# valida-xyz/valida

Measured on NVIDIA H100. Metric: trace rows/sec proven (Fibonacci), higher is better.
Workload: dtype u32 (BabyBear, 31-bit modular) + ext5

## Files before the change

### valida_b200/csrc/bb.cuh

```cuda
#pragma once
#include <cstdint>
#include <cuda_runtime.h>

namespace bb {

constexpr uint32_t P = 0x78000001u;
constexpr uint32_t PINV = 0x88000001u;
constexpr uint32_t R1 = 0x0ffffffeu;
constexpr uint32_t R2 = 1172168163u;
constexpr uint32_t GEN_CANON = 31;

#ifdef __CUDACC__
#define BB_HD __host__ __device__ __forceinline__
#else
#define BB_HD inline
#endif

BB_HD uint32_t umin32(uint32_t a, uint32_t b) { return a < b ? a : b; }
BB_HD uint32_t add(uint32_t a, uint32_t b) { uint32_t s = a + b; return umin32(s, s - P); }
BB_HD uint32_t sub(uint32_t a, uint32_t b) { uint32_t d = a - b; return umin32(d, d + P); }
BB_HD uint32_t neg(uint32_t a) { return a ? P - a : 0; }
BB_HD uint32_t dbl(uint32_t a) { return add(a, a); }
BB_HD uint32_t mul(uint32_t a, uint32_t b) {
    uint64_t t = (uint64_t)a * b;
    uint32_t m = (uint32_t)t * PINV;
#ifdef __CUDA_ARCH__
    uint32_t u = (uint32_t)(t >> 32) - __umulhi(m, P);
#else
    uint32_t u = (uint32_t)(t >> 32) - (uint32_t)(((uint64_t)m * P) >> 32);
#endif
    return umin32(u, u + P);
}
BB_HD uint32_t sqr(uint32_t a) { return mul(a, a); }
BB_HD uint32_t to_monty(uint32_t canonical) { return mul(canonical, R2); }
BB_HD uint32_t from_monty(uint32_t m) { return mul(m, 1u); }
BB_HD uint32_t pow(uint32_t a_monty, uint64_t e) {
    uint32_t r = R1;
    while (e) { if (e & 1) r = mul(r, a_monty); a_monty = mul(a_monty, a_monty); e >>= 1; }
    return r;
}
BB_HD uint32_t inv(uint32_t a_monty) { return pow(a_monty, P - 2); }

struct E5 { uint32_t c[5]; };
BB_HD E5 e5_zero() { E5 r; for (int i = 0; i < 5; i++) r.c[i] = 0; return r; }
BB_HD E5 e5_one() { E5 r = e5_zero(); r.c[0] = R1; return r; }
BB_HD E5 e5_from_base(uint32_t b) { E5 r = e5_zero(); r.c[0] = b; return r; }
BB_HD bool e5_is_zero(const E5& a) { return (a.c[0] | a.c[1] | a.c[2] | a.c[3] | a.c[4]) == 0; }
BB_HD E5 e5_add(const E5& a, const E5& b) { E5 r; for (int i = 0; i < 5; i++) r.c[i] = add(a.c[i], b.c[i]); return r; }
BB_HD E5 e5_sub(const E5& a, const E5& b) { E5 r; for (int i = 0; i < 5; i++) r.c[i] = sub(a.c[i], b.c[i]); return r; }
BB_HD E5 e5_neg(const E5& a) { E5 r; for (int i = 0; i < 5; i++) r.c[i] = neg(a.c[i]); return r; }
BB_HD E5 e5_add_base(const E5& a, uint32_t b) { E5 r = a; r.c[0] = add(r.c[0], b); return r; }
BB_HD E5 e5_sub_base(const E5& a, uint32_t b) { E5 r = a; r.c[0] = sub(r.c[0], b); return r; }
BB_HD E5 e5_mul_base(const E5& a, uint32_t b) { E5 r; for (int i = 0; i < 5; i++) r.c[i] = mul(a.c[i], b); return r; }

BB_HD uint32_t monty_reduce64(uint64_t t) {
    uint32_t hi = (uint32_t)(t >> 32), lo = (uint32_t)t;
    hi = umin32(hi, hi - P); hi = umin32(hi, hi - P);
    uint32_t m = lo * PINV;
#ifdef __CUDA_ARCH__
    uint32_t u = hi - __umulhi(m, P);
#else
    uint32_t u = hi - (uint32_t)(((uint64_t)m * P) >> 32);
#endif
    return umin32(u, u + P);
}

#ifdef __CUDACC__
__device__ __forceinline__ uint64_t madw(uint32_t a, uint32_t b, uint64_t c) {
    uint64_t r;
    asm("mad.wide.u32 %0, %1, %2, %3;" : "=l"(r) : "r"(a), "r"(b), "l"(c));
    return r;
}
__device__ __forceinline__ uint64_t lazy_fold(uint64_t a) { return madw((uint32_t)(a >> 32), R1, (uint64_t)(uint32_t)a); }

struct Lazy5 {
    uint64_t a[5]; int np;
    __device__ __forceinline__ void init() { for (int l = 0; l < 5; l++) a[l] = 0; np = 0; }
    __device__ __forceinline__ void fold() { for (int l = 0; l < 5; l++) a[l] = lazy_fold(a[l]); np = 0; }
    __device__ __forceinline__ void step() { if (np == 4) fold(); np++; }
    __device__ __forceinline__ void fma_base(const E5& x, uint32_t y) {
        step();
#pragma unroll
        for (int l = 0; l < 5; l++) a[l] = madw(x.c[l], y, a[l]);
    }
    __device__ __forceinline__ void fma_ext(const E5& x, const E5& y, const E5& y2) {
#pragma unroll
        for (int r = 0; r < 5; r++) {
            step();
#pragma unroll
            for (int k = 0; k < 5; k++) a[k] = madw(x.c[r], k >= r ? y.c[k - r] : y2.c[k - r + 5], a[k]);
        }
    }
    __device__ __forceinline__ E5 value() const { E5 r; for (int l = 0; l < 5; l++) r.c[l] = monty_reduce64(a[l]); return r; }
};
__device__ __forceinline__ E5 e5_dbl(const E5& a) { E5 r; for (int i = 0; i < 5; i++) r.c[i] = dbl(a.c[i]); return r; }
#endif

BB_HD E5 e5_mul(const E5& a, const E5& b) {
#ifdef __CUDA_ARCH__
    Lazy5 t; t.init(); t.fma_ext(a, b, e5_dbl(b));
    return t.value();
#else
    E5 r;
#define PR(i, j) ((uint64_t)a.c[i] * b.c[j])
    uint32_t l0 = monty_reduce64(PR(0, 0));
    uint32_t l1 = monty_reduce64(PR(0, 1) + PR(1, 0));
    uint32_t l2 = monty_reduce64(PR(0, 2) + PR(1, 1) + PR(2, 0));
    uint32_t l3 = monty_reduce64(PR(0, 3) + PR(1, 2) + PR(2, 1) + PR(3, 0));
    uint32_t l4 = add(monty_reduce64(PR(0, 4) + PR(1, 3) + PR(2, 2) + PR(3, 1)), monty_reduce64(PR(4, 0)));
    uint32_t h0 = monty_reduce64(PR(1, 4) + PR(2, 3) + PR(3, 2) + PR(4, 1));
    uint32_t h1 = monty_reduce64(PR(2, 4) + PR(3, 3) + PR(4, 2));
    uint32_t h2 = monty_reduce64(PR(3, 4) + PR(4, 3));
    uint32_t h3 = monty_reduce64(PR(4, 4));
#undef PR
    r.c[0] = add(l0, dbl(h0));
    r.c[1] = add(l1, dbl(h1));
    r.c[2] = add(l2, dbl(h2));
    r.c[3] = add(l3, dbl(h3));
    r.c[4] = l4;
    return r;
#endif
}
BB_HD E5 e5_sqr(const E5& a) { return e5_mul(a, a); }
BB_HD E5 e5_pow(E5 a, uint64_t e) {
    E5 r = e5_one();
    while (e) { if (e & 1) r = e5_mul(r, a); a = e5_sqr(a); e >>= 1; }
    return r;
}
BB_HD E5 e5_exp_pow2(E5 a, int k) { while (k-- > 0) a = e5_sqr(a); return a; }
BB_HD E5 e5_frobenius(const E5& a, const uint32_t zpow[5]) {
    E5 r; r.c[0] = a.c[0];
    for (int i = 1; i < 5; i++) r.c[i] = mul(a.c[i], zpow[i]);
    return r;
}
BB_HD void e5_frob_consts(uint32_t zpow[5]) {
    uint32_t z = pow(to_monty(2), (P - 1) / 5);
    zpow[0] = R1;
    for (int i = 1; i < 5; i++) zpow[i] = mul(zpow[i - 1], z);
}
BB_HD E5 e5_inv(const E5& a) {
    uint32_t zp[5];
    e5_frob_consts(zp);
    E5 f1 = e5_frobenius(a, zp), f2 = e5_frobenius(f1, zp), f3 = e5_frobenius(f2, zp), f4 = e5_frobenius(f3, zp);
    E5 prod = e5_mul(e5_mul(f1, f2), e5_mul(f3, f4));
    E5 n = e5_mul(a, prod);
    return e5_mul_base(prod, inv(n.c[0]));
}

BB_HD uint32_t reverse_bits(uint32_t x, int bits) {
#ifdef __CUDA_ARCH__
    return bits ? (__brev(x) >> (32 - bits)) : 0;
#else
    uint32_t r = 0;
    for (int i = 0; i < bits; i++) r = (r << 1) | ((x >> i) & 1);
    return r;
#endif
}

BB_HD uint32_t two_adic_generator_monty(int bits) {
    uint32_t g = to_monty(0x1a427a41u);
    for (int i = 0; i < 27 - bits; i++) g = sqr(g);
    return g;
}

}
```

### valida_b200/csrc/ntt.cu

```cuda
#include "ctx.h"
#include <cstdlib>

namespace {

using bb::mul; using bb::add; using bb::sub;

struct PassParams {
    const uint32_t* src; uint32_t* dst;
    uint64_t src_cs, dst_cs;
    uint64_t src_rs, src_gs;
    uint64_t dst_rs, dst_gs;
    uint32_t log_len;
    uint32_t tile;
    uint64_t groups;
    uint32_t inverse;
    uint32_t src_bitrev;
    uint32_t dst_natural;
    uint32_t g_bits;
    uint32_t pre_mode; uint32_t pre_r, pre_g, pre_shift;
    uint32_t post_mode; uint32_t post_shift, post_g, post_k; uint32_t post_scale;
    const uint32_t* root_lo; const uint32_t* root_hi;
    const uint32_t* root3;
    const uint32_t* tab_lo; const uint32_t* tab_hi;
    uint32_t tab_base;
    uint32_t tab_step;
};

__device__ __forceinline__ uint32_t root_pow(const PassParams& p, uint32_t e) {
    const uint32_t a = __ldg(p.root3 + (e & 511)), b = __ldg(p.root3 + 512 + ((e >> 9) & 511)), c = __ldg(p.root3 + 1024 + ((e >> 18) & 511));
    return mul(mul(a, b), c);
}

__device__ __forceinline__ uint32_t pad(uint32_t i) { return i + (i >> 4) + (i >> 9); }

template <int LQ, int RHO>
__device__ __forceinline__ constexpr uint32_t unit_off(uint32_t m) {
    uint32_t o = m << LQ;
    o += (LQ >= 4) ? (m << (LQ >= 4 ? LQ - 4 : 0)) : (m >> (LQ < 4 ? 4 - LQ : 0));
    if (LQ >= 9) o += m << (LQ >= 9 ? LQ - 9 : 0);
    else if (LQ + RHO >= 9) o += m >> (LQ < 9 ? 9 - LQ : 0);
    return o;
}

template <int RHO, int LOG_LEN, int S>
__device__ __forceinline__ void radix_unit(uint32_t* __restrict__ grp, const uint32_t* __restrict__ tw, uint32_t u) {
    constexpr int R = 1 << RHO;
    constexpr int LQ = LOG_LEN - S - RHO;
    constexpr bool IMM = (LQ + RHO >= 4);
    const uint32_t j = u & ((1u << LQ) - 1), blk = u >> LQ;
    const uint32_t base = (blk << (LQ + RHO)) + j;
    uint32_t* const g0 = grp + pad(base);
    uint32_t x[R];
#pragma unroll
    for (int m = 0; m < R; m++) x[m] = IMM ? g0[unit_off<LQ, RHO>(m)] : grp[pad(base + ((uint32_t)m << LQ))];
#pragma unroll
    for (int a = 0; a < RHO; a++) {
        const int half = R >> (a + 1);
        constexpr int E0 = LQ + S;
        const uint32_t tj = j << (S + a);
        const uint32_t* const tw0 = tw + tj + (tj >> 5);
#pragma unroll
        for (int m0 = 0; m0 < R; m0++) {
            if ((m0 & half) == 0) {
                const int m1 = m0 + half, mm = m0 & (half - 1);
                const uint32_t A = x[m0], B = x[m1];
                x[m0] = add(A, B);
                if (a == RHO - 1 && LQ == 0) x[m1] = sub(A, B);
                else {
                    const uint32_t d = A - B + bb::P;
                    uint32_t wv;
                    if (E0 + a >= 5) wv = tw0[((uint32_t)mm << (E0 + a)) + ((uint32_t)mm << (E0 + a >= 5 ? E0 + a - 5 : 0))];
                    else { const uint32_t ti = tj + ((uint32_t)mm << (E0 + a)); wv = tw[ti + (ti >> 5)]; }
                    x[m1] = mul(d, wv);
                }
            }
        }
    }
#pragma unroll
    for (int m = 0; m < R; m++) { if (IMM) g0[unit_off<LQ, RHO>(m)] = x[m]; else grp[pad(base + ((uint32_t)m << LQ))] = x[m]; }
}

template <int RHO, int LOG_LEN, int S>
__device__ __forceinline__ void radix_step(uint32_t* data, const uint32_t* tw, uint32_t T, uint32_t LS, uint32_t tid, uint32_t nt) {
    constexpr int LU = LOG_LEN - RHO;
    const uint32_t total_units = T << LU;
    for (uint32_t w = tid; w < total_units; w += nt) {
        const uint32_t t = w >> LU, u = w & ((1u << LU) - 1);
        radix_unit<RHO, LOG_LEN, S>(data + t * LS, tw, u);
    }
    __syncthreads();
}

template <int LOG_LEN, int S>
__device__ __forceinline__ void all_stages(uint32_t* data, const uint32_t* tw, uint32_t T, uint32_t LS, uint32_t tid, uint32_t nt) {
    if constexpr (LOG_LEN - S >= 4) {
        radix_step<4, LOG_LEN, S>(data, tw, T, LS, tid, nt);
        all_stages<LOG_LEN, S + 4>(data, tw, T, LS, tid, nt);
    } else if constexpr (LOG_LEN - S == 3) {
        radix_step<3, LOG_LEN, S>(data, tw, T, LS, tid, nt);
    } else if constexpr (LOG_LEN - S == 2) {
        radix_step<2, LOG_LEN, S>(data, tw, T, LS, tid, nt);
    } else if constexpr (LOG_LEN - S == 1) {
        radix_step<1, LOG_LEN, S>(data, tw, T, LS, tid, nt);
    }
}

__host__ __device__ constexpr uint32_t cbrev(uint32_t x, int bits) {
    uint32_t r = 0;
    for (int i = 0; i < bits; i++) r |= ((x >> i) & 1u) << (bits - 1 - i);
    return r;
}
template <int LOG_LEN> struct Std {
    static constexpr int LOG_T = 14 - LOG_LEN;
    static constexpr uint32_t T = 1u << (LOG_T > 0 ? LOG_T : 0), L = 1u << LOG_LEN;
    static constexpr uint32_t LS = (L + (L >> 4) + (L >> 9)) | 1;
    static constexpr int LR0 = LOG_LEN - 5;
    static constexpr int LB = LOG_LEN - 9;
};
__device__ __forceinline__ constexpr uint32_t off_b5(uint32_t c) { return c + (c >> 4); }
template <int LR0> __device__ __forceinline__ constexpr uint32_t off_strided(uint32_t k) {
    return (k << LR0) + (LR0 >= 4 ? (k << (LR0 >= 4 ? LR0 - 4 : 0)) : (k >> (LR0 < 4 ? 4 - LR0 : 0))) + (k >> (9 - LR0));
}
template <int LR0> __device__ __forceinline__ uint32_t base_strided(uint32_t r0) { return r0 + (LR0 >= 4 ? (r0 >> 4) : 0u); }
template <int LB> __device__ __forceinline__ uint32_t base_rowrev(uint32_t B) { return (B << LB) + ((B << LB) >> 4) + (B >> (9 - LB)); }
template <int LB> __device__ __forceinline__ constexpr uint32_t off_rowrev(uint32_t c) { return c + (LB >= 4 ? (c >> 4) : 0u); }

template <int LOG_LEN, bool BITREV>
__device__ __forceinline__ void load_strided_std(const PassParams& p, const uint32_t* __restrict__ src, uint32_t* __restrict__ data, uint64_t g0, uint32_t tid) {
    using S = Std<LOG_LEN>;
    const uint32_t tt = tid & (S::T - 1), r0 = tid >> S::LOG_T;
    const uint32_t* g = src + g0 + tt + (uint64_t)r0 * p.src_rs;
    const uint64_t ks = p.src_rs << S::LR0;
    uint32_t* sl;
    if (BITREV) { const uint32_t B = bb::reverse_bits(r0, S::LR0); sl = data + tt * S::LS + (B << 5) + (B << 1) + (B >> 4); }
    else sl = data + tt * S::LS + base_strided<S::LR0>(r0);
#pragma unroll
    for (int kb = 0; kb < 32; kb += 8) {
        uint32_t v[8];
#pragma unroll
        for (int u = 0; u < 8; u++) v[u] = __ldg(g + (uint64_t)(kb + u) * ks);
#pragma unroll
        for (int u = 0; u < 8; u++) sl[BITREV ? off_b5(cbrev(kb + u, 5)) : off_strided<S::LR0>(kb + u)] = v[u];
    }
}
template <int LOG_LEN, bool BITREV>
__device__ __forceinline__ void load_rows_std(const PassParams& p, const uint32_t* __restrict__ src, uint32_t* __restrict__ data, uint64_t g0, uint32_t tid) {
    using S = Std<LOG_LEN>;
    constexpr uint32_t I = 1u << S::LB;
    const uint32_t sb = BITREV ? base_rowrev<S::LB>(bb::reverse_bits(tid, 9)) : tid + (tid >> 4);
#pragma unroll
    for (uint32_t t = 0; t < S::T; t++) {
        const uint32_t* g = src + (g0 + t) * p.src_gs + tid;
        uint32_t* sl = data + t * S::LS + sb;
#pragma unroll
        for (uint32_t kb = 0; kb < I; kb += 8) {
            uint32_t v[8];
#pragma unroll
            for (uint32_t u = 0; u < 8 && kb + u < I; u++) v[u] = __ldg(g + 512 * (kb + u));
#pragma unroll
            for (uint32_t u = 0; u < 8 && kb + u < I; u++) sl[BITREV ? off_rowrev<S::LB>(cbrev(kb + u, S::LB)) : (kb + u) * 545u] = v[u];
        }
    }
}

template <int LOG_LEN>
__device__ __forceinline__ void load_rows_odd_std(const PassParams& p, const uint32_t* __restrict__ src, uint32_t* __restrict__ data, uint64_t g0, uint32_t tid) {
    using S = Std<LOG_LEN>;
    constexpr uint32_t I = 1u << S::LB;
    const uint32_t B = bb::reverse_bits(tid, 9);
    const uint32_t sb = base_rowrev<S::LB>(B);
    const uint32_t step = root_pow(p, p.pre_r << p.pre_shift);
#pragma unroll 8
    for (uint32_t t = 0; t < S::T; t++) {
        const uint32_t g = (uint32_t)g0 + t;
        const uint32_t gval = p.g_bits ? bb::reverse_bits(g, (int)p.g_bits) : g;
        uint32_t m = root_pow(p, (((B << S::LB) * p.pre_r) + gval * p.pre_g) << p.pre_shift);
        const uint32_t* gp = src + (uint64_t)g * p.src_gs + tid;
        uint32_t* sl = data + t * S::LS + sb;
#pragma unroll
        for (uint32_t ib = 0; ib < I; ib += 8) {
            uint32_t v[8];
#pragma unroll
            for (uint32_t u = 0; u < 8 && ib + u < I; u++) v[u] = __ldg(gp + 512 * cbrev(ib + u, S::LB));
#pragma unroll
            for (uint32_t u = 0; u < 8 && ib + u < I; u++) { sl[off_rowrev<S::LB>(ib + u)] = mul(v[u], m); m = mul(m, step); }
        }
    }
}

__device__ __forceinline__ void post_begin(const PassParams& p, uint32_t gval, uint32_t k_start, uint32_t k_stride, uint32_t* m, uint32_t* step) {
    if (p.post_mode == 1) {
        uint32_t e0 = (gval * k_start) << p.post_shift, es = (gval * k_stride) << p.post_shift;
        if (p.inverse) { e0 = 0u - e0; es = 0u - es; }
        *m = root_pow(p, e0); *step = root_pow(p, es);
    } else if (p.post_mode == 2) {
        const uint32_t e0 = gval * p.post_g + k_start * p.post_k;
        *m = mul(__ldg(p.tab_lo + (e0 & (VG_POW_LO - 1))), __ldg(p.tab_hi + (e0 >> VG_POW_LO_BITS)));
        *step = p.tab_step;
    } else { *m = p.post_mode == 3 ? p.post_scale : bb::R1; *step = bb::R1; }
}
template <int LOG_LEN, bool NAT>
__device__ __forceinline__ void store_rows_std(const PassParams& p, uint32_t* __restrict__ dst, const uint32_t* __restrict__ data, uint64_t g0, uint32_t tid) {
    using S = Std<LOG_LEN>;
    constexpr uint32_t I = 1u << S::LB;
    const uint32_t B = bb::reverse_bits(tid, 9);
    const uint32_t sb = NAT ? base_rowrev<S::LB>(B) : tid + (tid >> 4);
    const bool running = p.post_mode == 1 || p.post_mode == 2;
#pragma unroll
    for (uint32_t t = 0; t < S::T; t++) {
        const uint32_t g = (uint32_t)g0 + t;
        const uint32_t gval = p.g_bits ? bb::reverse_bits(g, (int)p.g_bits) : g;
        uint32_t m, step;
        post_begin(p, gval, NAT ? tid : (B << S::LB), NAT ? 512u : 1u, &m, &step);
        uint32_t* d = dst + (uint64_t)g * p.dst_gs + tid;
        const uint32_t* sl = data + t * S::LS + sb;
#pragma unroll
        for (uint32_t i = 0; i < I; i++) {
            const uint32_t j = NAT ? i : cbrev(i, S::LB);
            const uint32_t v = sl[NAT ? off_rowrev<S::LB>(cbrev(i, S::LB)) : j * 545u];
            d[512 * j] = p.post_mode ? mul(v, m) : v;
            if (running) m = mul(m, step);
        }
    }
}
template <int LOG_LEN, bool NAT>
__device__ __forceinline__ void store_short_rows_std(const PassParams& p, uint32_t* __restrict__ dst, const uint32_t* __restrict__ data, uint64_t g0, uint32_t tid) {
    using S = Std<LOG_LEN>;
    constexpr uint32_t GPS = 512u >> LOG_LEN;
    const uint32_t pos = tid & (S::L - 1), t0 = tid >> LOG_LEN;
    const uint32_t q = NAT ? bb::reverse_bits(pos, LOG_LEN) : pos;
    uint32_t* d = dst + (g0 + t0) * p.dst_gs + pos;
    const uint64_t ks = p.dst_gs * GPS;
    const uint32_t* sl = data + t0 * S::LS + pad(q);
#pragma unroll
    for (uint32_t kb = 0; kb < 32; kb += 8) {
        uint32_t v[8];
#pragma unroll
        for (uint32_t u = 0; u < 8; u++) v[u] = sl[(kb + u) * GPS * S::LS];
#pragma unroll
        for (uint32_t u = 0; u < 8; u++) d[(uint64_t)(kb + u) * ks] = p.post_mode == 3 ? mul(v[u], p.post_scale) : v[u];
    }
}
template <int LOG_LEN, bool NAT>
__device__ __forceinline__ void store_strided_std(const PassParams& p, uint32_t* __restrict__ dst, const uint32_t* __restrict__ data, uint64_t g0, uint32_t tid) {
    using S = Std<LOG_LEN>;
    const uint32_t tt = tid & (S::T - 1), r0 = tid >> S::LOG_T;
    const uint32_t g = (uint32_t)g0 + tt;
    const uint32_t gval = p.g_bits ? bb::reverse_bits(g, (int)p.g_bits) : g;
    const uint32_t Bq = bb::reverse_bits(r0, S::LR0);
    uint32_t m, step;
    post_begin(p, gval, NAT ? r0 : (Bq << 5), NAT ? (1u << S::LR0) : 1u, &m, &step);
    const bool running = p.post_mode == 1 || p.post_mode == 2;
    uint32_t* d = dst + g + (uint64_t)r0 * p.dst_rs;
    const uint64_t ks = p.dst_rs << S::LR0;
    const uint32_t* sl = data + tt * S::LS + (NAT ? (Bq << 5) + (Bq << 1) + (Bq >> 4) : base_strided<S::LR0>(r0));
#pragma unroll
    for (uint32_t i = 0; i < 32; i++) {
        const uint32_t j = NAT ? i : cbrev(i, 5);
        const uint32_t v = sl[NAT ? off_b5(cbrev(i, 5)) : off_strided<S::LR0>(j)];
        d[(uint64_t)j * ks] = p.post_mode ? mul(v, m) : v;
        if (running) m = mul(m, step);
    }
}

template <int LOG_LEN>
__global__ void __launch_bounds__(512) ntt_pass_kernel(PassParams p) {
    extern __shared__ uint32_t smem[];
    constexpr uint32_t L = 1u << LOG_LEN;
    const uint32_t T = p.tile;
    const uint32_t LS = (L + (L >> 4) + (L >> 9)) | 1;
    uint32_t* tw = smem;
    uint32_t* data = smem + (L >= 2 ? L / 2 + L / 64 + 1 : 1);
    const uint32_t tid = threadIdx.x, nt = blockDim.x;
    const uint64_t col = blockIdx.y;
    const uint64_t g0 = (uint64_t)blockIdx.x * T;
    const uint32_t* src = p.src + col * p.src_cs;
    uint32_t* dst = p.dst + col * p.dst_cs;

    {
        const uint64_t unit = (1ull << VG_LOG_NMAX) >> LOG_LEN;
        for (uint32_t j = tid; j < L / 2; j += nt) {
            uint64_t e = (uint64_t)j * unit;
            if (p.inverse && e) e = (1ull << VG_LOG_NMAX) - e;
            tw[j + (j >> 5)] = __ldg(p.root_hi + (e >> VG_POW_LO_BITS));
        }
    }
    const uint32_t total = L * T;
    const uint32_t log_t = 31 - __clz(T);
    bool std_shape = false, loaded = false;
    if constexpr (LOG_LEN >= 8 && LOG_LEN <= 14) {
        std_shape = (T == Std<LOG_LEN>::T) && nt == 512;
        if constexpr (LOG_LEN >= 9) {
            if (std_shape && p.pre_mode && p.src_bitrev && p.src_rs == 1 && p.src_gs != 1) { load_rows_odd_std<LOG_LEN>(p, src, data, g0, tid); loaded = true; }
        }
        if (std_shape && !p.pre_mode) {
            if constexpr (LOG_LEN <= 12) {
                if (p.src_gs == 1) {
                    if (p.src_bitrev) load_strided_std<LOG_LEN, true>(p, src, data, g0, tid); else load_strided_std<LOG_LEN, false>(p, src, data, g0, tid);
                    loaded = true;
                }
            }
            if constexpr (LOG_LEN >= 9) {
                if (!loaded && p.src_rs == 1 && p.src_gs != 1) {
                    if (p.src_bitrev) load_rows_std<LOG_LEN, true>(p, src, data, g0, tid); else load_rows_std<LOG_LEN, false>(p, src, data, g0, tid);
                    loaded = true;
                }
            }
        }
    }
    if (!loaded) {
        const bool tfast = (p.src_gs == 1);
        const uint32_t log_nt = 31 - __clz(nt);
        if (p.pre_mode && p.src_bitrev && !tfast && L >= 4 * nt) {
            const uint32_t ibits = LOG_LEN - log_nt, I = 1u << ibits;
            const uint32_t r_start = bb::reverse_bits(tid, (int)log_nt) << ibits;
            const uint32_t step = root_pow(p, p.pre_r << p.pre_shift);
            const uint32_t step2 = mul(step, step), step3 = mul(step2, step), step4 = mul(step2, step2);
            for (uint32_t t = 0; t < T; t++) {
                const uint32_t g = (uint32_t)g0 + t;
                const uint32_t gval = p.g_bits ? bb::reverse_bits(g, (int)p.g_bits) : g;
                uint32_t m = root_pow(p, (r_start * p.pre_r + gval * p.pre_g) << p.pre_shift);
                const uint32_t* srow = src + (uint64_t)g * p.src_gs;
                uint32_t* drow = data + t * LS;
                for (uint32_t i = 0; i < I; i += 4) {
                    uint32_t v[4];
#pragma unroll
                    for (int u = 0; u < 4; u++) v[u] = srow[tid + (bb::reverse_bits(i + u, (int)ibits) << log_nt)];
                    drow[pad(r_start + i)] = mul(v[0], m);
                    drow[pad(r_start + i + 1)] = mul(v[1], mul(m, step));
                    drow[pad(r_start + i + 2)] = mul(v[2], mul(m, step2));
                    drow[pad(r_start + i + 3)] = mul(v[3], mul(m, step3));
                    m = mul(m, step4);
                }
            }
        } else
        for (uint32_t idx0 = tid; idx0 < total; idx0 += 4 * nt) {
            uint32_t v[4], tt[4], rr[4];
#pragma unroll
            for (int u = 0; u < 4; u++) {
                const uint32_t idx = idx0 + u * nt;
                if (idx < total) {
                    if (tfast) { tt[u] = idx & (T - 1); rr[u] = idx >> log_t; } else { rr[u] = idx & (L - 1); tt[u] = idx >> LOG_LEN; }
                    v[u] = src[(uint64_t)rr[u] * p.src_rs + (g0 + tt[u]) * p.src_gs];
                }
            }
#pragma unroll
            for (int u = 0; u < 4; u++) {
                const uint32_t idx = idx0 + u * nt;
                if (idx < total) {
                    const uint32_t rnat = p.src_bitrev ? bb::reverse_bits(rr[u], (int)LOG_LEN) : rr[u];
                    uint32_t x = v[u];
                    if (p.pre_mode) {
                        const uint32_t g = (uint32_t)g0 + tt[u];
                        const uint32_t gval = p.g_bits ? bb::reverse_bits(g, (int)p.g_bits) : g;
                        x = mul(x, root_pow(p, (rnat * p.pre_r + gval * p.pre_g) << p.pre_shift));
                    }
                    data[tt[u] * LS + pad(rnat)] = x;
                }
            }
        }
    }
    __syncthreads();
    all_stages<LOG_LEN, 0>(data, tw, T, LS, tid, nt);
    bool stored = false;
    if constexpr (LOG_LEN >= 8 && LOG_LEN <= 14) {
        if (std_shape) {
            if constexpr (LOG_LEN <= 12) {
                if (p.dst_gs == 1) {
                    if (p.dst_natural) store_strided_std<LOG_LEN, true>(p, dst, data, g0, tid); else store_strided_std<LOG_LEN, false>(p, dst, data, g0, tid);
                    stored = true;
                }
            }
            if (!stored && p.dst_rs == 1 && p.dst_gs != 1) {
                if constexpr (LOG_LEN >= 9) {
                    if (p.dst_natural) store_rows_std<LOG_LEN, true>(p, dst, data, g0, tid); else store_rows_std<LOG_LEN, false>(p, dst, data, g0, tid);
                    stored = true;
                } else {
                    if (p.post_mode == 0 || p.post_mode == 3) {
                        if (p.dst_natural) store_short_rows_std<LOG_LEN, true>(p, dst, data, g0, tid); else store_short_rows_std<LOG_LEN, false>(p, dst, data, g0, tid);
                        stored = true;
                    }
                }
            }
        }
    }
    if (!stored) {
        const bool tfast = (p.dst_gs == 1);
        const uint32_t log_nt = 31 - __clz(nt);
        const bool fast = tfast ? (nt >= T && log_nt - log_t <= (uint32_t)LOG_LEN) : (L >= nt);
        if (fast && (p.post_mode == 1 || p.post_mode == 2)) {
            const uint32_t lowbits = tfast ? (log_nt - log_t) : log_nt;
            const uint32_t ibits = LOG_LEN - lowbits, I = 1u << ibits;
            const uint32_t p0 = tfast ? (tid >> log_t) : tid;
            const uint32_t ngroups_here = tfast ? 1u : T;
            for (uint32_t tg = 0; tg < ngroups_here; tg++) {
                const uint32_t t = tfast ? (tid & (T - 1)) : tg;
                const uint32_t g = (uint32_t)g0 + t;
                const uint32_t gval = p.g_bits ? bb::reverse_bits(g, (int)p.g_bits) : g;
                const uint32_t k_start = p.dst_natural ? p0 : (bb::reverse_bits(p0, (int)lowbits) << ibits);
                const uint32_t k_stride = p.dst_natural ? (1u << lowbits) : 1u;
                uint32_t m, step;
                if (p.post_mode == 1) {
                    uint32_t e0 = (gval * k_start) << p.post_shift, es = (gval * k_stride) << p.post_shift;
                    if (p.inverse) { e0 = 0u - e0; es = 0u - es; }
                    m = root_pow(p, e0); step = root_pow(p, es);
                } else {
                    const uint32_t e0 = gval * p.post_g + k_start * p.post_k;
                    m = mul(__ldg(p.tab_lo + (e0 & (VG_POW_LO - 1))), __ldg(p.tab_hi + (e0 >> VG_POW_LO_BITS)));
                    step = p.tab_step;
                }
                uint32_t* dcol = dst + (uint64_t)g * p.dst_gs;
                const uint32_t* drow = data + t * LS;
                for (uint32_t i = 0; i < I; i++) {
                    const uint32_t j = p.dst_natural ? i : bb::reverse_bits(i, (int)ibits);
                    const uint32_t pos = p0 + (j << lowbits);
                    const uint32_t q = p.dst_natural ? bb::reverse_bits(pos, (int)LOG_LEN) : pos;
                    dcol[(uint64_t)pos * p.dst_rs] = mul(drow[pad(q)], m);
                    m = mul(m, step);
                }
            }
        } else {
            for (uint32_t idx = tid; idx < total; idx += nt) {
                uint32_t t, pos;
                if (tfast) { t = idx & (T - 1); pos = idx >> log_t; } else { pos = idx & (L - 1); t = idx >> LOG_LEN; }
                const uint32_t brp = bb::reverse_bits(pos, (int)LOG_LEN);
                const uint32_t q = p.dst_natural ? brp : pos;
                const uint32_t k = p.dst_natural ? pos : brp;
                uint32_t v = data[t * LS + pad(q)];
                if (p.post_mode) {
                    const uint32_t g = (uint32_t)g0 + t;
                    const uint32_t gval = p.g_bits ? bb::reverse_bits(g, (int)p.g_bits) : g;
                    if (p.post_mode == 1) {
                        uint32_t e = (gval * k) << p.post_shift;
                        if (p.inverse) e = (0u - e);
                        v = mul(v, root_pow(p, e));
                    } else if (p.post_mode == 2) {
                        const uint32_t e = gval * p.post_g + k * p.post_k;
                        v = mul(v, mul(__ldg(p.tab_lo + (e & (VG_POW_LO - 1))), __ldg(p.tab_hi + (e >> VG_POW_LO_BITS))));
                    } else {
                        v = mul(v, p.post_scale);
                    }
                }
                dst[(uint64_t)pos * p.dst_rs + (g0 + t) * p.dst_gs] = v;
            }
        }
    }
}

constexpr int LOG_ROW_MAX = 14;
constexpr int LOG_COL_MAX = 12;
constexpr int LOG_TILE_ELEMS = 14;

uint32_t choose_tile(int log_len, uint64_t groups) {
    int lt = LOG_TILE_ELEMS - log_len;
    if (lt < 0) lt = 0;
    if (lt > 6) lt = 6;
    uint32_t t = 1u << lt;
    while (t > groups) t >>= 1;
    return t ? t : 1;
}

int32_t launch_pass(vgpu_ctx* ctx, PassParams p, uint64_t w) {
    p.root_lo = ctx->root_table.lo; p.root_hi = ctx->root_table.hi; p.root3 = ctx->root3;
    const uint32_t L = 1u << p.log_len;
    p.tile = choose_tile((int)p.log_len, p.groups);
    const uint64_t tiles = p.groups / p.tile;
    const uint32_t LS = (L + (L >> 4) + (L >> 9)) | 1;
    const size_t smem = ((L >= 2 ? L / 2 + L / 64 + 1 : 1) + (size_t)p.tile * LS) * sizeof(uint32_t);
    const uint32_t total = L * p.tile;
    uint32_t threads = total / 16 >= 512 ? 512 : (total / 16 >= 32 ? total / 16 : 32);
    if (total >= (1u << 14) && threads > 256) threads = 256 * 2;
    using KernelFn = void (*)(PassParams);
    static const KernelFn kernels[15] = {ntt_pass_kernel<0>, ntt_pass_kernel<1>, ntt_pass_kernel<2>, ntt_pass_kernel<3>, ntt_pass_kernel<4>, ntt_pass_kernel<5>,
                                         ntt_pass_kernel<6>, ntt_pass_kernel<7>, ntt_pass_kernel<8>, ntt_pass_kernel<9>, ntt_pass_kernel<10>, ntt_pass_kernel<11>,
                                         ntt_pass_kernel<12>, ntt_pass_kernel<13>, ntt_pass_kernel<14>};
    if (p.log_len > 14) VG_FAIL(ctx, "ntt: sub-transform 2^%u exceeds the shared-memory tile", p.log_len);
    if (!ctx->ntt_attrs_set) { for (auto k : kernels) VG_CUDA(ctx, cudaFuncSetAttribute(k, cudaFuncAttributeMaxDynamicSharedMemorySize, 200 * 1024)); ctx->ntt_attrs_set = true; }
    if (p.post_mode == 2) {
        uint32_t log_nt = 0; while ((1u << log_nt) < threads) log_nt++;
        uint32_t log_t = 0; while ((1u << log_t) < p.tile) log_t++;
        const bool tfast = (p.dst_gs == 1);
        const uint32_t lowbits = tfast ? (log_nt >= log_t ? log_nt - log_t : 0) : log_nt;
        const uint64_t k_stride = p.dst_natural ? (1ull << lowbits) : 1ull;
        p.tab_step = bb::pow(p.tab_base, k_stride * p.post_k);
    }
    for (uint64_t c0 = 0; c0 < w; c0 += 65535) {
        const uint64_t wc = w - c0 < 65535 ? w - c0 : 65535;
        PassParams q = p;
        q.src = p.src + c0 * p.src_cs; q.dst = p.dst + c0 * p.dst_cs;
        dim3 grid((unsigned)tiles, (unsigned)wc);
        KScope ks(ctx, KC_NTT, 8.0 * (double)(p.groups << p.log_len) * (double)wc);
        kernels[p.log_len]<<<grid, threads, smem, ctx->stream>>>(q);
        VG_LAUNCH_CHECK(ctx);
    }
    return 0;
}

__global__ void repeat_row_kernel(const uint32_t* src, uint64_t src_cs, uint32_t* dst, uint64_t dst_cs, uint64_t H, uint64_t w) {
    uint64_t i = (uint64_t)blockIdx.x * blockDim.x + threadIdx.x;
    if (i >= H * w) return;
    dst[(i / H) * dst_cs + (i % H)] = src[(i / H) * src_cs];
}

__global__ void zero_pad_kernel(const uint32_t* src, uint64_t src_cs, uint32_t* dst, uint64_t dst_cs, uint64_t h, uint64_t H, uint64_t w) {
    uint64_t i = (uint64_t)blockIdx.x * blockDim.x + threadIdx.x;
    if (i >= H * w) return;
    uint64_t c = i / H, r = i % H;
    dst[c * dst_cs + r] = r < h ? src[c * src_cs + r] : 0;
}

void split_col_row(int log_n, int* l_col, int* l_row) {
    if (log_n <= LOG_ROW_MAX) { *l_col = 0; *l_row = log_n; return; }
    static const int row_split = [] { const char* e = getenv("VGPU_NTT_LOG_ROW"); int v = e ? atoi(e) : LOG_ROW_MAX; return v < 8 || v > LOG_ROW_MAX ? LOG_ROW_MAX : v; }();
    int lc = log_n - row_split;
    if (lc > LOG_COL_MAX) lc = LOG_COL_MAX;
    if (lc < 4) lc = 4;
    *l_col = lc; *l_row = log_n - lc;
}

}

int32_t vg_ntt_nat2nat(vgpu_ctx* ctx, const uint32_t* src, uint64_t src_cs, uint32_t* dst, uint64_t dst_cs, int log_n, uint64_t w,
                       bool inverse, const PowTable* coset, uint32_t* tmp, uint64_t tmp_cs) {
    const uint64_t n = 1ull << log_n;
    uint32_t ninv = inverse ? bb::inv(bb::to_monty((uint32_t)(n % bb::P))) : bb::R1;
    PassParams p{};
    p.inverse = inverse;
    if (log_n <= LOG_ROW_MAX) {
        p.src = src; p.src_cs = src_cs; p.dst = dst; p.dst_cs = dst_cs;
        p.src_rs = 1; p.src_gs = n; p.dst_rs = 1; p.dst_gs = n;
        p.log_len = log_n; p.groups = 1; p.dst_natural = 1;
        if (coset) { p.post_mode = 2; p.post_g = 0; p.post_k = 1; p.tab_lo = coset->lo; p.tab_hi = coset->hi; p.tab_base = coset->base; }
        else if (inverse) { p.post_mode = 3; p.post_scale = ninv; }
        return launch_pass(ctx, p, w);
    }
    if (log_n > VG_LOG_NMAX) VG_FAIL(ctx, "ntt: 2^%d exceeds BabyBear's two-adicity (2^%d)", log_n, VG_LOG_NMAX);
    const int l1 = (log_n + 1) / 2, l2 = log_n - l1;
    const uint64_t n1 = 1ull << l1, n2 = 1ull << l2;
    p.src = src; p.src_cs = src_cs; p.dst = tmp; p.dst_cs = tmp_cs;
    p.src_rs = n2; p.src_gs = 1; p.dst_rs = 1; p.dst_gs = n1;
    p.log_len = l1; p.groups = n2; p.dst_natural = 1;
    p.post_mode = 1; p.post_shift = VG_LOG_NMAX - log_n;
    VG_TRY(launch_pass(ctx, p, w));
    PassParams q{};
    q.inverse = inverse;
    q.src = tmp; q.src_cs = tmp_cs; q.dst = dst; q.dst_cs = dst_cs;
    q.src_rs = n1; q.src_gs = 1; q.dst_rs = n1; q.dst_gs = 1;
    q.log_len = l2; q.groups = n1; q.dst_natural = 1;
    if (coset) { q.post_mode = 2; q.post_g = 1; q.post_k = (uint32_t)n1; q.tab_lo = coset->lo; q.tab_hi = coset->hi; q.tab_base = coset->base; }
    else if (inverse) { q.post_mode = 3; q.post_scale = ninv; }
    return launch_pass(ctx, q, w);
}

static int32_t intt_nat2bitrev_scaled(vgpu_ctx* ctx, const uint32_t* src, uint64_t src_cs, uint32_t* buf, uint64_t bcs, int log_n, uint64_t w, const PowTable* tab) {
    const uint64_t n = 1ull << log_n;
    int lc, lr;
    split_col_row(log_n, &lc, &lr);
    PassParams p{};
    p.inverse = 1;
    if (lc == 0) {
        p.src = src; p.src_cs = src_cs; p.dst = buf; p.dst_cs = bcs;
        p.src_rs = 1; p.src_gs = n; p.dst_rs = 1; p.dst_gs = n;
        p.log_len = log_n; p.groups = 1; p.dst_natural = 0;
        p.post_mode = 2; p.post_g = 0; p.post_k = 1; p.tab_lo = tab->lo; p.tab_hi = tab->hi; p.tab_base = tab->base;
        return launch_pass(ctx, p, w);
    }
    const uint64_t n1 = 1ull << lc, n2 = 1ull << lr;
    p.src = src; p.src_cs = src_cs; p.dst = buf; p.dst_cs = bcs;
    p.src_rs = n2; p.src_gs = 1; p.dst_rs = n2; p.dst_gs = 1;
    p.log_len = lc; p.groups = n2; p.dst_natural = 0;
    p.post_mode = 1; p.post_shift = VG_LOG_NMAX - log_n;
    VG_TRY(launch_pass(ctx, p, w));
    PassParams q{};
    q.inverse = 1;
    q.src = buf; q.src_cs = bcs; q.dst = buf; q.dst_cs = bcs;
    q.src_rs = 1; q.src_gs = n2; q.dst_rs = 1; q.dst_gs = n2;
    q.log_len = lr; q.groups = n1; q.dst_natural = 0;
    q.g_bits = lc;
    q.post_mode = 2; q.post_g = 1; q.post_k = (uint32_t)n1; q.tab_lo = tab->lo; q.tab_hi = tab->hi; q.tab_base = tab->base;
    return launch_pass(ctx, q, w);
}

static int32_t ntt_bitrev2bitrev(vgpu_ctx* ctx, const uint32_t* coef, uint64_t ccs, uint32_t* dst, uint64_t dst_cs, uint32_t* tmp, uint64_t tcs,
                                 int log_n, uint64_t w, bool odd, bool inverse = false, const PowTable* tab = nullptr) {
    const uint64_t n = 1ull << log_n;
    int lc, lr;
    split_col_row(log_n, &lc, &lr);
    PassParams p{};
    p.inverse = inverse ? 1 : 0;
    if (lc == 0) {
        p.src = coef; p.src_cs = ccs; p.dst = dst; p.dst_cs = dst_cs;
        p.src_rs = 1; p.src_gs = n; p.dst_rs = 1; p.dst_gs = n;
        p.log_len = log_n; p.groups = 1; p.src_bitrev = 1; p.dst_natural = 0;
        if (odd) { p.pre_mode = 1; p.pre_r = 1; p.pre_g = 0; p.pre_shift = VG_LOG_NMAX - (log_n + 1); }
        if (tab) { p.post_mode = 2; p.post_g = 0; p.post_k = 1; p.tab_lo = tab->lo; p.tab_hi = tab->hi; p.tab_base = tab->base; }
        return launch_pass(ctx, p, w);
    }
    const uint64_t n1 = 1ull << lc, n2 = 1ull << lr;
    p.src = coef; p.src_cs = ccs; p.dst = tmp; p.dst_cs = tcs;
    p.src_rs = 1; p.src_gs = n2; p.dst_rs = 1; p.dst_gs = n2;
    p.log_len = lr; p.groups = n1; p.src_bitrev = 1; p.dst_natural = 0;
    p.g_bits = lc;
    if (odd) { p.pre_mode = 1; p.pre_r = (uint32_t)n1; p.pre_g = 1; p.pre_shift = VG_LOG_NMAX - (log_n + 1); }
    p.post_mode = 1; p.post_shift = VG_LOG_NMAX - log_n;
    VG_TRY(launch_pass(ctx, p, w));
    PassParams q{};
    q.inverse = inverse ? 1 : 0;
    q.src = tmp; q.src_cs = tcs; q.dst = dst; q.dst_cs = dst_cs;
    q.src_rs = n2; q.src_gs = 1; q.dst_rs = 1; q.dst_gs = n1;
    q.log_len = lc; q.groups = n2; q.src_bitrev = 1; q.dst_natural = 0;
    if (tab) {
        q.g_bits = lr; q.post_mode = 2; q.post_g = 1; q.post_k = (uint32_t)n2;
        q.tab_lo = tab->lo; q.tab_hi = tab->hi; q.tab_base = tab->base;
    }
    return launch_pass(ctx, q, w);
}

int32_t vg_coset_lde(vgpu_ctx* ctx, const uint32_t* src, uint64_t src_cs, uint64_t h, uint64_t w, uint32_t shift_canonical,
                     uint32_t* dst, uint64_t dst_cs, bool bit_reversed, bool src_bitrev, uint32_t log_blowup) {
    if (src_bitrev && !bit_reversed) VG_FAIL(ctx, "coset_lde: a bit-reversed-row input is only supported with bit-reversed output");
    if (bit_reversed && log_blowup != 1) VG_FAIL(ctx, "coset_lde: committed (bit-reversed) extensions are built for log_blowup = 1 only (FriConfig of basic/src/bin/valida.rs:385-390)");
    int log_n = 0;
    while ((1ull << log_n) < h) log_n++;
    if ((1ull << log_n) != h) VG_FAIL(ctx, "coset_lde: height %llu is not a power of two", (unsigned long long)h);
    if (log_n + (int)log_blowup > VG_LOG_NMAX) VG_FAIL(ctx, "coset_lde: LDE height 2^%d exceeds BabyBear two-adicity", log_n + (int)log_blowup);
    if (log_n > LOG_ROW_MAX + LOG_COL_MAX) VG_FAIL(ctx, "coset_lde: heights above 2^%d are not built", LOG_ROW_MAX + LOG_COL_MAX);
    if (h == 1) {
        const uint64_t H = 1ull << log_blowup;
        repeat_row_kernel<<<(unsigned)((H * w + 127) / 128), 128, 0, ctx->stream>>>(src, src_cs, dst, dst_cs, H, w);
        VG_LAUNCH_CHECK(ctx);
        return 0;
    }
    const PowTable* tab = nullptr;
    uint32_t ninv_canon = bb::from_monty(bb::inv(bb::to_monty((uint32_t)(h % bb::P))));
    VG_TRY(vg_get_shift_table(ctx, shift_canonical, ninv_canon, h, &tab));
    uint64_t batch = (2ull << 30) / (8 * h);
    if (batch < 1) batch = 1;
    if (batch > w) batch = w;
    uint32_t *coef = nullptr, *tmp = nullptr;
    VG_TRY(vg_alloc(ctx, (void**)&coef, batch * h * 4));
    VG_TRY(vg_alloc(ctx, (void**)&tmp, batch * h * 4));
    int32_t rc = 0;
    for (uint64_t c0 = 0; c0 < w && rc == 0; c0 += batch) {
        uint64_t wc = w - c0 < batch ? w - c0 : batch;
        if (bit_reversed) {
            rc = src_bitrev ? ntt_bitrev2bitrev(ctx, src + c0 * src_cs, src_cs, coef, h, tmp, h, log_n, wc, false, true, tab)
                            : intt_nat2bitrev_scaled(ctx, src + c0 * src_cs, src_cs, coef, h, log_n, wc, tab);
            if (rc) break;
            rc = ntt_bitrev2bitrev(ctx, coef, h, dst + c0 * dst_cs, dst_cs, tmp, h, log_n, wc, false);
            if (rc) break;
            rc = ntt_bitrev2bitrev(ctx, coef, h, dst + c0 * dst_cs + h, dst_cs, tmp, h, log_n, wc, true);
        } else {
            rc = vg_ntt_nat2nat(ctx, src + c0 * src_cs, src_cs, coef, h, log_n, wc, true, tab, tmp, h);
            if (rc) break;
            const uint64_t H = h << log_blowup;
            uint32_t* padb = nullptr; uint32_t* tmp2 = nullptr;
            rc = vg_alloc(ctx, (void**)&padb, wc * H * 4); if (rc) break;
            rc = vg_alloc(ctx, (void**)&tmp2, wc * H * 4); if (rc) { vg_free(ctx, padb); break; }
            uint64_t tot = H * wc;
            zero_pad_kernel<<<(unsigned)((tot + 255) / 256), 256, 0, ctx->stream>>>(coef, h, padb, H, h, H, wc);
            ctx->launches++;
            rc = vg_ntt_nat2nat(ctx, padb, H, dst + c0 * dst_cs, dst_cs, log_n + (int)log_blowup, wc, false, nullptr, tmp2, H);
            vg_free(ctx, padb); vg_free(ctx, tmp2);
        }
    }
    vg_free(ctx, coef); vg_free(ctx, tmp);
    return rc;
}
```

Measured before the change: 23.21 million.

## Use Shoup precomputed-quotient twiddle multiplication in shared-memory NTT stages

Replaces Montgomery multiplication by twiddles in the NTT butterflies with Shoup multiplication, storing each twiddle with its precomputed quotient as a uint2 in shared memory. For sub-transforms longer than 2^12, only stages from the fourth onward use Shoup twiddles and the first stage group keeps the old table, so the radix schedule is reordered to put the short radix step after the first radix-16 step. This saves one multiply-high per butterfly but roughly doubles the twiddle shared-memory footprint and adds per-block setup work to compute the quotients. A profiling script for the LDE is also added.

```diff
diff --git a/profiles/prof_lde.py b/profiles/prof_lde.py
--- /dev/null
+++ b/profiles/prof_lde.py
@@ -0,0 +1,33 @@
+import os
+import sys
+
+ROOT = os.path.dirname(os.path.dirname(os.path.abspath(__file__)))
+sys.path.insert(0, ROOT)
+import numpy as np
+import torch
+import valida_b200 as vb
+
+reps = int(sys.argv[1]) if len(sys.argv) > 1 else 10
+ctx = vb.Context(0)
+dft = vb.Radix2Dft(ctx)
+rng = np.random.default_rng(5)
+for log_h, w in ((24, 14), (22, 51), (22, 16)):
+    a = ctx.upload(rng.integers(0, vb.BABYBEAR_P, (1 << log_h, w), dtype=np.uint32))
+    del_ = dft.coset_lde_batch(a, 1, 31, bit_reversed=True)
+    del del_
+    ctx.synchronize()
+    ms = []
+    for _ in range(reps):
+        l0 = ctx.launch_count
+        e0, e1 = torch.cuda.Event(enable_timing=True), torch.cuda.Event(enable_timing=True)
+        ctx.synchronize()
+        e0.record()
+        out = dft.coset_lde_batch(a, 1, 31, bit_reversed=True)
+        ctx.synchronize()
+        e1.record()
+        e1.synchronize()
+        ms.append(e0.elapsed_time(e1))
+        launches = ctx.launch_count - l0
+        del out
+    print("lde 2^%d x %d: median %.3f ms, min %.3f ms, %d launches" % (log_h, w, float(np.median(ms)), min(ms), launches), flush=True)
+    del a
diff --git a/valida_b200/csrc/bb.cuh b/valida_b200/csrc/bb.cuh
--- a/valida_b200/csrc/bb.cuh
+++ b/valida_b200/csrc/bb.cuh
@@ -30,6 +30,16 @@
     uint32_t u = (uint32_t)(t >> 32) - (uint32_t)(((uint64_t)m * P) >> 32);
 #endif
     return umin32(u, u + P);
+}
+BB_HD uint32_t shoup_quot(uint32_t w) { return (uint32_t)(((uint64_t)w << 32) / P); }
+BB_HD uint32_t mul_shoup(uint32_t d, uint32_t w, uint32_t wq) {
+#ifdef __CUDA_ARCH__
+    const uint32_t q = __umulhi(d, wq);
+#else
+    const uint32_t q = (uint32_t)(((uint64_t)d * wq) >> 32);
+#endif
+    const uint32_t r = d * w - q * P;
+    return umin32(r, r - P);
 }
 BB_HD uint32_t sqr(uint32_t a) { return mul(a, a); }
 BB_HD uint32_t to_monty(uint32_t canonical) { return mul(canonical, R2); }
diff --git a/valida_b200/csrc/ntt.cu b/valida_b200/csrc/ntt.cu
--- a/valida_b200/csrc/ntt.cu
+++ b/valida_b200/csrc/ntt.cu
@@ -42,8 +42,15 @@
     return o;
 }
 
+constexpr int LOG_SHOUP_ALL = 12;
+__host__ __device__ constexpr int shoup_from(int log_len) { return log_len > LOG_SHOUP_ALL ? 4 : 0; }
+__host__ __device__ constexpr uint32_t shoup_entries(int log_len) { return log_len >= 1 ? (1u << (log_len - 1)) >> shoup_from(log_len) : 0u; }
+__host__ __device__ constexpr uint32_t twiddle_words(int log_len) {
+    return 2 * (shoup_entries(log_len) + shoup_entries(log_len) / 16) + (shoup_from(log_len) ? (1u << (log_len - 1)) + (1u << log_len) / 64 + 1 : 0u);
+}
+
 template <int RHO, int LOG_LEN, int S>
-__device__ __forceinline__ void radix_unit(uint32_t* __restrict__ grp, const uint32_t* __restrict__ tw, uint32_t u) {
+__device__ __forceinline__ void radix_unit(uint32_t* __restrict__ grp, const uint32_t* __restrict__ tw, const uint2* __restrict__ sh, uint32_t u) {
     constexpr int R = 1 << RHO;
     constexpr int LQ = LOG_LEN - S - RHO;
     constexpr bool IMM = (LQ + RHO >= 4);
@@ -66,7 +73,15 @@
                 const uint32_t A = x[m0], B = x[m1];
                 x[m0] = add(A, B);
                 if (a == RHO - 1 && LQ == 0) x[m1] = sub(A, B);
-                else {
+                else if (S + a >= shoup_from(LOG_LEN)) {
+                    constexpr int SH = shoup_from(LOG_LEN);
+                    const int EK = E0 + a - SH;
+                    const uint32_t tk = j << (S + a - SH);
+                    uint2 wv;
+                    if (EK >= 4) wv = sh[tk + (tk >> 4) + ((uint32_t)mm << EK) + ((uint32_t)mm << (EK >= 4 ? EK - 4 : 0))];
+                    else { const uint32_t k = tk + ((uint32_t)mm << EK); wv = sh[k + (k >> 4)]; }
+                    x[m1] = bb::mul_shoup(A - B + bb::P, wv.x, wv.y);
+                } else {
                     const uint32_t d = A - B + bb::P;
                     uint32_t wv;
                     if (E0 + a >= 5) wv = tw0[((uint32_t)mm << (E0 + a)) + ((uint32_t)mm << (E0 + a >= 5 ? E0 + a - 5 : 0))];
@@ -81,27 +96,26 @@
 }
 
 template <int RHO, int LOG_LEN, int S>
-__device__ __forceinline__ void radix_step(uint32_t* data, const uint32_t* tw, uint32_t T, uint32_t LS, uint32_t tid, uint32_t nt) {
+__device__ __forceinline__ void radix_step(uint32_t* data, const uint32_t* tw, const uint2* sh, uint32_t T, uint32_t LS, uint32_t tid, uint32_t nt) {
     constexpr int LU = LOG_LEN - RHO;
     const uint32_t total_units = T << LU;
     for (uint32_t w = tid; w < total_units; w += nt) {
         const uint32_t t = w >> LU, u = w & ((1u << LU) - 1);
-        radix_unit<RHO, LOG_LEN, S>(data + t * LS, tw, u);
+        radix_unit<RHO, LOG_LEN, S>(data + t * LS, tw, sh, u);
     }
     __syncthreads();
 }
 
+__host__ __device__ constexpr int step_radix(int log_len, int s) {
+    return (log_len % 4 != 0 && s == (shoup_from(log_len) ? 4 : 0)) ? log_len % 4 : 4;
+}
+
 template <int LOG_LEN, int S>
-__device__ __forceinline__ void all_stages(uint32_t* data, const uint32_t* tw, uint32_t T, uint32_t LS, uint32_t tid, uint32_t nt) {
-    if constexpr (LOG_LEN - S >= 4) {
-        radix_step<4, LOG_LEN, S>(data, tw, T, LS, tid, nt);
-        all_stages<LOG_LEN, S + 4>(data, tw, T, LS, tid, nt);
-    } else if constexpr (LOG_LEN - S == 3) {
-        radix_step<3, LOG_LEN, S>(data, tw, T, LS, tid, nt);
-    } else if constexpr (LOG_LEN - S == 2) {
-        radix_step<2, LOG_LEN, S>(data, tw, T, LS, tid, nt);
-    } else if constexpr (LOG_LEN - S == 1) {
-        radix_step<1, LOG_LEN, S>(data, tw, T, LS, tid, nt);
+__device__ __forceinline__ void all_stages(uint32_t* data, const uint32_t* tw, const uint2* sh, uint32_t T, uint32_t LS, uint32_t tid, uint32_t nt) {
+    if constexpr (S < LOG_LEN) {
+        constexpr int RHO = step_radix(LOG_LEN, S);
+        radix_step<RHO, LOG_LEN, S>(data, tw, sh, T, LS, tid, nt);
+        all_stages<LOG_LEN, S + RHO>(data, tw, sh, T, LS, tid, nt);
     }
 }
 
@@ -269,8 +283,11 @@
     constexpr uint32_t L = 1u << LOG_LEN;
     const uint32_t T = p.tile;
     const uint32_t LS = (L + (L >> 4) + (L >> 9)) | 1;
-    uint32_t* tw = smem;
-    uint32_t* data = smem + (L >= 2 ? L / 2 + L / 64 + 1 : 1);
+    constexpr int SH = shoup_from(LOG_LEN);
+    constexpr uint32_t NSH = shoup_entries(LOG_LEN);
+    uint2* sh = reinterpret_cast<uint2*>(smem);
+    uint32_t* tw = smem + 2 * (NSH + NSH / 16);
+    uint32_t* data = smem + twiddle_words(LOG_LEN);
     const uint32_t tid = threadIdx.x, nt = blockDim.x;
     const uint64_t col = blockIdx.y;
     const uint64_t g0 = (uint64_t)blockIdx.x * T;
@@ -279,10 +296,18 @@
 
     {
         const uint64_t unit = (1ull << VG_LOG_NMAX) >> LOG_LEN;
-        for (uint32_t j = tid; j < L / 2; j += nt) {
-            uint64_t e = (uint64_t)j * unit;
+        if constexpr (SH > 0) {
+            for (uint32_t j = tid; j < L / 2; j += nt) {
+                uint64_t e = (uint64_t)j * unit;
+                if (p.inverse && e) e = (1ull << VG_LOG_NMAX) - e;
+                tw[j + (j >> 5)] = __ldg(p.root_hi + (e >> VG_POW_LO_BITS));
+            }
+        }
+        for (uint32_t k = tid; k < NSH; k += nt) {
+            uint64_t e = ((uint64_t)k << SH) * unit;
             if (p.inverse && e) e = (1ull << VG_LOG_NMAX) - e;
-            tw[j + (j >> 5)] = __ldg(p.root_hi + (e >> VG_POW_LO_BITS));
+            const uint32_t w = bb::from_monty(__ldg(p.root_hi + (e >> VG_POW_LO_BITS)));
+            sh[k + (k >> 4)] = make_uint2(w, bb::shoup_quot(w));
         }
     }
     const uint32_t total = L * T;
@@ -361,7 +386,7 @@
         }
     }
     __syncthreads();
-    all_stages<LOG_LEN, 0>(data, tw, T, LS, tid, nt);
+    all_stages<LOG_LEN, 0>(data, tw, sh, T, LS, tid, nt);
     bool stored = false;
     if constexpr (LOG_LEN >= 8 && LOG_LEN <= 14) {
         if (std_shape) {
@@ -466,7 +491,7 @@
     p.tile = choose_tile((int)p.log_len, p.groups);
     const uint64_t tiles = p.groups / p.tile;
     const uint32_t LS = (L + (L >> 4) + (L >> 9)) | 1;
-    const size_t smem = ((L >= 2 ? L / 2 + L / 64 + 1 : 1) + (size_t)p.tile * LS) * sizeof(uint32_t);
+    const size_t smem = (twiddle_words((int)p.log_len) + (size_t)p.tile * LS) * sizeof(uint32_t);
     const uint32_t total = L * p.tile;
     uint32_t threads = total / 16 >= 512 ? 512 : (total / 16 >= 32 ? total / 16 : 32);
     if (total >= (1u << 14) && threads > 256) threads = 256 * 2;
```

After: 23.45 million, median of 6. 1.01x the previous value.
